# voutcn/megahit

Measured on NVIDIA H100. Metric: sorted (k+1)-mer edges/sec at k=27 on 150bp reads, higher is better.
Workload: dtype u32

## Files before the change

### megahit_b200/csrc/mhb_part.cuh

```cuda
#pragma once
#include "mhb_sort3.cuh"

namespace mhb {

__device__ __forceinline__ u32 atom_shared_inc_ret(u32 *p) {
  u32 old;
  asm volatile("atom.shared.add.u32 %0, [%1], 1;" : "=r"(old) : "r"(smem_u32(p)) : "memory");
  return old;
}

template <int WR>
struct PartCfg {
  static constexpr int THREADS = 384;
  static constexpr int IPT = SortGeom<WR>::IPT;
  static constexpr int TILE = THREADS * IPT;
  static constexpr size_t SMEM = 256 * 8  + 4 * 256 * 4  + 16 * 4 + (size_t)TILE * WR * 4;
  static constexpr size_t SMEM_OWNER_HIST = SMEM + 16 * 256 * 4;
};

template <int WR, bool OWNER_LUT, bool HAS_NEXT>
__global__ void __launch_bounds__(PartCfg<WR>::THREADS, 2)
    k_part_unstable(const u32 *__restrict__ in, u64 n, u32 num_tiles, int byte_idx,
                    const u64 *__restrict__ bin_addr ,
                    unsigned long long *gcursor , u32 *tile_counter,
                    u64 *next_hist, int next_byte, const uint8_t *__restrict__ digit_lut) {
  constexpr bool OWNER_HIST = OWNER_LUT && HAS_NEXT;
  using C = PartCfg<WR>;
  constexpr int THREADS = C::THREADS, IPT = C::IPT, TILE = C::TILE;
  extern __shared__ __align__(16) unsigned char smem_raw[];
  u64 *s_base = reinterpret_cast<u64 *>(smem_raw);
  u32 *s_cnt = reinterpret_cast<u32 *>(s_base + 256);
  u32 *s_off = s_cnt + 256;
  u32 *s_cur = s_off + 256;
  u32 *s_next = s_cur + 256;
  u32 *s_misc = s_next + 256;
  u32 *s_recs = s_misc + 16;
  u32 *s_onext = s_recs + (size_t)C::TILE * WR;
  __shared__ uint8_t s_lut[OWNER_LUT ? 256 : 1];
  const u32 tid = threadIdx.x, lane = tid & 31, warp = tid >> 5;
  const u32 widx = (u32)(WR - 1 - (byte_idx >> 2)), bsel = (u32)(byte_idx & 3);
  const u32 nwidx = (u32)(WR - 1 - (next_byte >> 2)), nbsel = (u32)(next_byte & 3);
  for (int i = tid; i < 256; i += THREADS) {
    s_cnt[i] = 0;
    s_next[i] = 0;
  }
  if constexpr (OWNER_HIST) {
    for (int i = tid; i < 16 * 256; i += THREADS) s_onext[i] = 0;
  }
  if constexpr (OWNER_LUT) {
    for (int i = tid; i < 256; i += THREADS) s_lut[i] = digit_lut[i];
  }
  if (tid == 0) s_misc[0] = atomicAdd(tile_counter, 1u);
  __syncthreads();
  u32 tile = s_misc[0];
  while (tile < num_tiles) {
    u32 next_ticket = 0;
    if (tid == 0) next_ticket = atomicAdd(tile_counter, 1u);
    const u64 tile_base = (u64)tile * TILE;
    const u32 valid = tile_base + TILE <= n ? (u32)TILE : (u32)(n - tile_base);
    u32 r[IPT][WR];
    u32 dg[IPT];
    const u32 wbase = warp * 32 * IPT + lane;
#pragma unroll
    for (int i = 0; i < IPT; ++i) {
      const u32 p = wbase + (u32)i * 32;
      if (p < valid) ld_rec_pinned<WR>(in, tile_base + p, r[i]);
    }
#pragma unroll
    for (int i = 0; i < IPT; ++i) {
      const u32 p = wbase + (u32)i * 32;
      u32 d = 0;
      if (p < valid) {
        d = rec_digit<WR>(r[i], widx, bsel);
        if constexpr (OWNER_LUT) d = s_lut[d];
        red_shared_inc(&s_cnt[d]);
      }
      dg[i] = d;
    }
    __syncthreads();
    if (tid < 256) {
      const u32 c = s_cnt[tid];
      const unsigned long long g = c ? atomicAdd(&gcursor[tid], (unsigned long long)c) : 0ull;
      u32 inc = c;
#pragma unroll
      for (int dd = 1; dd < 32; dd <<= 1) {
        const u32 t = __shfl_up_sync(0xffffffffu, inc, dd);
        if (lane >= (u32)dd) inc += t;
      }
      if (lane == 31) s_misc[4 + warp] = inc;
      s_off[tid] = inc - c;
      s_base[tid] = bin_addr[tid] + g * (u64)(WR * 4);
    }
    __syncthreads();
    if (tid < 256) {
      u32 add = 0;
#pragma unroll
      for (int w = 0; w < 7; ++w) add += (warp > (u32)w) ? s_misc[4 + w] : 0u;
      const u32 o = s_off[tid] + add;
      s_off[tid] = o;
      s_cur[tid] = o;
    }
    if (tid == 0) s_misc[0] = next_ticket;
    __syncthreads();
#pragma unroll
    for (int i = 0; i < IPT; ++i) {
      const u32 p = wbase + (u32)i * 32;
      if (p < valid) st_shared_rec<WR>(s_recs, atom_shared_inc_ret(&s_cur[dg[i]]), r[i]);
    }
    __syncthreads();
    const u32 next_tile = s_misc[0];
#pragma unroll
    for (int i = 0; i < IPT; ++i) {
      const u32 p = (u32)i * THREADS + tid;
      if (p < valid) {
        u32 q[WR];
        ld_rec<WR>(s_recs, p, q);
        u32 dd = rec_digit<WR>(q, widx, bsel);
        if constexpr (OWNER_LUT) dd = s_lut[dd];
        st_global_rec<WR>(s_base[dd] + (u64)(p - s_off[dd]) * (WR * 4), q);
        if constexpr (OWNER_HIST) red_shared_inc(&s_onext[(dd & 15u) * 256 + rec_digit<WR>(q, nwidx, nbsel)]);
        else if constexpr (HAS_NEXT) red_shared_inc(&s_next[rec_digit<WR>(q, nwidx, nbsel)]);
      }
    }
    for (int i = tid; i < 256; i += THREADS) s_cnt[i] = 0;
    __syncthreads();
    tile = next_tile;
  }
  if constexpr (OWNER_HIST) {
    for (int i = tid; i < 16 * 256; i += THREADS)
      if (s_onext[i]) atomicAdd((unsigned long long *)&next_hist[i], (unsigned long long)s_onext[i]);
  } else if constexpr (HAS_NEXT) {
    for (int i = tid; i < 256; i += THREADS)
      if (s_next[i]) atomicAdd((unsigned long long *)&next_hist[i], (unsigned long long)s_next[i]);
  }
}

}
```

### megahit_b200/csrc/mhb_sortdisp.cu

```cuda
#include <cuda_runtime.h>
#include <stdio.h>
#include <stdlib.h>
#include <string.h>

#include "mhb.h"
#include "mhb_common.cuh"
#include "mhb_kernels.cuh"
#include "mhb_sort3.cuh"
#include "mhb_part.cuh"

using namespace mhb;

template <int WR>
static u64 sort_tiles(u64 n) {
  return (n + SortGeom<WR>::TILE - 1) / SortGeom<WR>::TILE;
}
static u64 sort_num_tiles(u64 n, u32 words) {
#define M(WW) \
  if (words == WW) return sort_tiles<WW>(n);
  MHB_FOR_WR(M)
#undef M
  return 0;
}
static constexpr size_t kSortHeadBytes = (size_t)(72 + 1) * 256 * 8  + 256 * 8  + 128 * 4 + 256 * 8 ;

extern "C" size_t mhb_sort_workspace_bytes(uint64_t n, uint32_t words) {
  return kSortHeadBytes + (size_t)sort_num_tiles(n, words) * 256 * 8 + 256;
}

template <int WR>
static int launch_radix_pass(cudaStream_t st, const u32 *in, u64 n, int byte_idx, const u64 *bin_base,
                             u64 *lookback, u32 *tile_counter, u64 *next_hist, int next_byte, u32 epoch) {
  using G = SortGeom<WR>;
  static int blocks_per_sm = 0;
  if (!blocks_per_sm) {
    CK(cudaFuncSetAttribute(k_radix_pass3<WR, true>, cudaFuncAttributeMaxDynamicSharedMemorySize, (int)G::SMEM));
    CK(cudaFuncSetAttribute(k_radix_pass3<WR, false>, cudaFuncAttributeMaxDynamicSharedMemorySize, (int)G::SMEM));
    CK(cudaOccupancyMaxActiveBlocksPerMultiprocessor(&blocks_per_sm, k_radix_pass3<WR, true>, G::THREADS, G::SMEM));
    if (blocks_per_sm < 1) return mhb_set_error(MHB_ERR_CUDA, "radix pass kernel (WR=%d) does not fit an SM", WR);
    if (getenv("MHB_VERBOSE")) fprintf(stderr, "[mhb] radix pass WR=%d: %d threads x %d rec, %zu B smem, %d CTA/SM\n", WR, G::THREADS, G::IPT, G::SMEM, blocks_per_sm);
  }
  const u64 tiles = sort_tiles<WR>(n);
  u64 grid = (u64)blocks_per_sm * sm_count();
  if (grid > tiles) grid = tiles;
  if (next_hist)
    k_radix_pass3<WR, true><<<(int)grid, G::THREADS, G::SMEM, st>>>(in, n, (u32)tiles, byte_idx, bin_base, lookback,
                                                                     tile_counter, next_hist, next_byte, epoch);
  else
    k_radix_pass3<WR, false><<<(int)grid, G::THREADS, G::SMEM, st>>>(in, n, (u32)tiles, byte_idx, bin_base, lookback,
                                                                      tile_counter, nullptr, 0, epoch);
  CK_LAUNCH();
  return MHB_OK;
}

template <int WR, bool OWNER_LUT>
static int launch_part_unstable(cudaStream_t st, const u32 *in, u64 n, int byte_idx, const u64 *bin_base,
                                unsigned long long *gcursor, u32 *tile_counter, u64 *next_hist, int next_byte,
                                const uint8_t *lut) {
  using C = PartCfg<WR>;
  constexpr size_t SMEM_HIST = OWNER_LUT ? C::SMEM_OWNER_HIST : C::SMEM;
  static int bps = 0;
  if (!bps) {
    CK(cudaFuncSetAttribute(k_part_unstable<WR, OWNER_LUT, true>, cudaFuncAttributeMaxDynamicSharedMemorySize, (int)SMEM_HIST));
    CK(cudaFuncSetAttribute(k_part_unstable<WR, OWNER_LUT, false>, cudaFuncAttributeMaxDynamicSharedMemorySize, (int)C::SMEM));
    CK(cudaOccupancyMaxActiveBlocksPerMultiprocessor(&bps, k_part_unstable<WR, OWNER_LUT, true>, C::THREADS, SMEM_HIST));
    if (bps < 1) return mhb_set_error(MHB_ERR_CUDA, "partition pass (WR=%d) does not fit an SM", WR);
    if (getenv("MHB_VERBOSE")) fprintf(stderr, "[mhb] unstable partition pass WR=%d owner=%d: %d threads x %d rec, %zu B smem, %d CTA/SM\n", WR, (int)OWNER_LUT, C::THREADS, C::IPT, SMEM_HIST, bps);
  }
  const u64 tiles = (n + C::TILE - 1) / C::TILE;
  u64 grid = (u64)bps * sm_count();
  if (grid > tiles) grid = tiles;
  if (next_hist)
    k_part_unstable<WR, OWNER_LUT, true><<<(int)grid, C::THREADS, SMEM_HIST, st>>>(in, n, (u32)tiles, byte_idx, bin_base, gcursor,
                                                                                   tile_counter, next_hist, next_byte, lut);
  else
    k_part_unstable<WR, OWNER_LUT, false><<<(int)grid, C::THREADS, C::SMEM, st>>>(in, n, (u32)tiles, byte_idx, bin_base, gcursor,
                                                                                  tile_counter, nullptr, 0, lut);
  CK_LAUNCH();
  return MHB_OK;
}

#ifdef MHB_SORT_TIMELINE
extern "C" int mhb_debug_set_sort_timeline(unsigned long long *dev_buf, unsigned long long rows) {
  CK(cudaMemcpyToSymbol(g_sort_timeline, &dev_buf, sizeof(dev_buf)));
  CK(cudaMemcpyToSymbol(g_sort_timeline_rows, &rows, sizeof(rows)));
  return MHB_OK;
}
#endif

namespace {
struct SortTrace {
  cudaEvent_t ev[74];
  bool created = false;
  uint32_t n_passes = 0, words = 0;
  uint64_t n = 0;
};
SortTrace g_trace[4];
uint64_t g_trace_seq = 0;
}

static int sort_records_core(void *stream, uint32_t *a, uint32_t *b, uint64_t n, uint32_t words, const uint8_t *bytes,
                             uint32_t n_bytes, const uint64_t *first_hist, void *ws, size_t ws_bytes, int *result_in_b,
                             double *pass_ms_host, int relaxed, bool trace);
int mhb_sort_records_impl(void *stream, uint32_t *a, uint32_t *b, uint64_t n, uint32_t words, const uint8_t *bytes,
                          uint32_t n_bytes, const uint64_t *first_hist, void *ws, size_t ws_bytes, int *result_in_b,
                          double *pass_ms_host) {
  return sort_records_core(stream, a, b, n, words, bytes, n_bytes, first_hist, ws, ws_bytes, result_in_b, pass_ms_host, 1, true);
}
int mhb_sort_records_ex(void *stream, uint32_t *a, uint32_t *b, uint64_t n, uint32_t words, const uint8_t *bytes,
                        uint32_t n_bytes, const uint64_t *first_hist, void *ws, size_t ws_bytes, int *result_in_b,
                        double *pass_ms_host, int relaxed) {
  return sort_records_core(stream, a, b, n, words, bytes, n_bytes, first_hist, ws, ws_bytes, result_in_b, pass_ms_host, relaxed, true);
}
int mhb_sort_records_untraced(void *stream, uint32_t *a, uint32_t *b, uint64_t n, uint32_t words, const uint8_t *bytes,
                              uint32_t n_bytes, const uint64_t *first_hist, void *ws, size_t ws_bytes, int *result_in_b) {
  return sort_records_core(stream, a, b, n, words, bytes, n_bytes, first_hist, ws, ws_bytes, result_in_b, nullptr, 1, false);
}
static int sort_records_core(void *stream, uint32_t *a, uint32_t *b, uint64_t n, uint32_t words, const uint8_t *bytes,
                             uint32_t n_bytes, const uint64_t *first_hist, void *ws, size_t ws_bytes, int *result_in_b,
                             double *pass_ms_host, int relaxed, bool trace) {
  if (pass_ms_host && !trace) return mhb_set_error(MHB_ERR_ARG, "per-pass times need a traced sort");
  if (words < 1 || words > 17 || n_bytes > 72 || !result_in_b)
    return mhb_set_error(MHB_ERR_ARG, "bad sort geometry (words=%u n_bytes=%u)", words, n_bytes);
  *result_in_b = 0;
  if (n == 0 || n_bytes == 0) return MHB_OK;
  if (ws_bytes < mhb_sort_workspace_bytes(n, words)) return mhb_set_error(MHB_ERR_ARG, "sort workspace too small");
  if (n >= (1ull << 53)) return mhb_set_error(MHB_ERR_ARG, "too many records");
  cudaStream_t st = (cudaStream_t)stream;
  u64 *hist = (u64 *)ws;
  u64 *bin_base = hist + (72 + 1) * 256;
  u32 *tile_counter = (u32 *)(bin_base + 256);
  unsigned long long *gcursor = (unsigned long long *)(tile_counter + 128);
  u64 *lookback = (u64 *)((char *)ws + kSortHeadBytes);
  CK(cudaMemsetAsync(ws, 0, mhb_sort_workspace_bytes(n, words), st));
  if (first_hist) {
    CK(cudaMemcpyAsync(hist, first_hist, 256 * 8, cudaMemcpyDeviceToDevice, st));
  } else {
#define M(WW) \
  if (words == WW) k_hist_byte<WW><<<sm_count() * 4, 256, 0, st>>>(a, n, bytes[0], hist);
    MHB_FOR_WR(M)
#undef M
    CK_LAUNCH();
  }
  SortTrace *tr = nullptr;
  if (trace) {
    tr = &g_trace[g_trace_seq++ & 3];
    if (!tr->created) {
      for (int i = 0; i < 74; ++i) CK(cudaEventCreate(&tr->ev[i]));
      tr->created = true;
    }
    tr->n_passes = n_bytes;
    tr->words = words;
    tr->n = n;
    CK(cudaEventRecord(tr->ev[0], st));
  }
  u32 *in = a, *out = b;
  for (u32 p = 0; p < n_bytes; ++p) {
    k_hist_scan256<<<1, 256, 0, st>>>(hist + (u64)p * 256, bin_base, (u64)(uintptr_t)out, words * 4);
    CK_LAUNCH();
    u64 *next_hist = p + 1 < n_bytes ? hist + (u64)(p + 1) * 256 : nullptr;
    const int next_byte = p + 1 < n_bytes ? bytes[p + 1] : 0;
    int rc = MHB_ERR_ARG;
    if (p == 0 && relaxed && words == 2) rc = launch_part_unstable<2, false>(st, in, n, bytes[p], bin_base, gcursor, tile_counter + p, next_hist, next_byte, nullptr);
    else if (p == 0 && relaxed && words == 3) rc = launch_part_unstable<3, false>(st, in, n, bytes[p], bin_base, gcursor, tile_counter + p, next_hist, next_byte, nullptr);
    else {
#define M(WW) \
  if (words == WW) rc = launch_radix_pass<WW>(st, in, n, bytes[p], bin_base, lookback, tile_counter + p, next_hist, next_byte, p + 1);
      MHB_FOR_WR(M)
#undef M
    }
    if (rc) return rc;
    if (tr) CK(cudaEventRecord(tr->ev[p + 1], st));
    u32 *t = in;
    in = out;
    out = t;
  }
  *result_in_b = (in == b) ? 1 : 0;
  if (pass_ms_host) {
    CK(cudaEventSynchronize(tr->ev[n_bytes]));
    for (u32 p = 0; p < n_bytes; ++p) {
      float ms = 0;
      CK(cudaEventElapsedTime(&ms, tr->ev[p], tr->ev[p + 1]));
      pass_ms_host[p] = ms;
    }
  }
  return MHB_OK;
}

int hist_byte(void *stream, const uint32_t *recs, uint64_t n, uint32_t words, int byte, uint64_t *hist) {
  if (words < 1 || words > 17 || byte < 0 || byte >= (int)(4 * words)) return mhb_set_error(MHB_ERR_ARG, "bad geometry");
  if (n == 0) return MHB_OK;
  cudaStream_t st = (cudaStream_t)stream;
#define M(WW) \
  if (words == WW) k_hist_byte<WW><<<sm_count() * 4, 256, 0, st>>>(recs, n, byte, hist);
  MHB_FOR_WR(M)
#undef M
  CK_LAUNCH();
  return MHB_OK;
}

static int partition_scatter_impl(void *stream, const uint32_t *recs, uint64_t n, uint32_t words, int byte,
                                  const uint8_t *owner_of_byte_dev, const uint64_t *bin_addr_dev, void *ws, size_t ws_bytes,
                                  int next_byte, uint64_t *owner_next_hist) {
  if (words < 1 || words > 17 || byte < 0 || byte >= (int)(4 * words)) return mhb_set_error(MHB_ERR_ARG, "bad geometry");
  if (!owner_of_byte_dev) return mhb_set_error(MHB_ERR_ARG, "the partition pass needs an owner table");
  if (n == 0) return MHB_OK;
  if (ws_bytes < kSortHeadBytes) return mhb_set_error(MHB_ERR_ARG, "sort workspace too small");
  cudaStream_t st = (cudaStream_t)stream;
  u32 *tile_counter = (u32 *)((u64 *)ws + (72 + 1) * 256 + 256);
  unsigned long long *gcursor = (unsigned long long *)(tile_counter + 128);
  CK(cudaMemsetAsync(ws, 0, kSortHeadBytes, st));
  int rc = MHB_ERR_ARG;
#define M(WW)                                                                                                        \
  if (words == WW)                                                                                                   \
    rc = launch_part_unstable<WW, true>(st, recs, n, byte, bin_addr_dev, gcursor, tile_counter, owner_next_hist, next_byte, \
                                        owner_of_byte_dev);
  MHB_FOR_WR(M)
#undef M
  return rc;
}
extern "C" int mhb_partition_scatter(void *stream, const uint32_t *recs, uint64_t n, uint32_t words, int byte,
                                     const uint8_t *owner_of_byte_dev, const uint64_t *bin_addr_dev, void *ws,
                                     size_t ws_bytes) {
  return partition_scatter_impl(stream, recs, n, words, byte, owner_of_byte_dev, bin_addr_dev, ws, ws_bytes, 0, nullptr);
}
extern "C" int mhb_partition_scatter_hist(void *stream, const uint32_t *recs, uint64_t n, uint32_t words, int byte,
                                          const uint8_t *owner_of_byte_dev, const uint64_t *bin_addr_dev, void *ws,
                                          size_t ws_bytes, int next_byte, uint64_t *owner_next_hist) {
  if (!owner_next_hist || next_byte < 0 || next_byte >= (int)(4 * words))
    return mhb_set_error(MHB_ERR_ARG, "bad owner-histogram arguments");
  return partition_scatter_impl(stream, recs, n, words, byte, owner_of_byte_dev, bin_addr_dev, ws, ws_bytes, next_byte,
                                owner_next_hist);
}

extern "C" int mhb_dev_malloc(void **ptr, size_t bytes) {
  CK(cudaMalloc(ptr, bytes));
  return MHB_OK;
}
extern "C" int mhb_dev_free(void *ptr) {
  CK(cudaFree(ptr));
  return MHB_OK;
}
extern "C" int mhb_ipc_export(const void *dev_ptr, uint8_t *handle64) {
  static_assert(sizeof(cudaIpcMemHandle_t) == 64, "handle size");
  cudaIpcMemHandle_t h;
  CK(cudaIpcGetMemHandle(&h, const_cast<void *>(dev_ptr)));
  memcpy(handle64, &h, 64);
  return MHB_OK;
}
extern "C" int mhb_ipc_open(const uint8_t *handle64, void **peer_ptr) {
  cudaIpcMemHandle_t h;
  memcpy(&h, handle64, 64);
  CK(cudaIpcOpenMemHandle(peer_ptr, h, cudaIpcMemLazyEnablePeerAccess));
  return MHB_OK;
}
extern "C" int mhb_ipc_close(void *peer_ptr) {
  CK(cudaIpcCloseMemHandle(peer_ptr));
  return MHB_OK;
}

extern "C" int mhb_sort_pass_ms(int back, double *pass_ms, uint32_t max_passes, uint32_t *n_passes, uint64_t *n_records,
                                uint32_t *words) {
  if (back < 0 || back > 3 || (uint64_t)back >= g_trace_seq) return mhb_set_error(MHB_ERR_ARG, "no such sort in the trace ring");
  SortTrace &tr = g_trace[(g_trace_seq - 1 - back) & 3];
  CK(cudaEventSynchronize(tr.ev[tr.n_passes]));
  for (u32 p = 0; p < tr.n_passes && p < max_passes; ++p) {
    float ms = 0;
    CK(cudaEventElapsedTime(&ms, tr.ev[p], tr.ev[p + 1]));
    pass_ms[p] = ms;
  }
  if (n_passes) *n_passes = tr.n_passes;
  if (n_records) *n_records = tr.n;
  if (words) *words = tr.words;
  return MHB_OK;
}

extern "C" int mhb_sort_records(void *stream, uint32_t *a, uint32_t *b, uint64_t n, uint32_t words,
                                const uint8_t *bytes, uint32_t n_bytes, const uint64_t *first_hist, void *ws,
                                size_t ws_bytes, int *result_in_b) {
  return mhb_sort_records_ex(stream, a, b, n, words, bytes, n_bytes, first_hist, ws, ws_bytes, result_in_b, nullptr, 0);
}

extern "C" int mhb_sort_records_relaxed(void *stream, uint32_t *a, uint32_t *b, uint64_t n, uint32_t words,
                                        const uint8_t *bytes, uint32_t n_bytes, const uint64_t *first_hist, void *ws,
                                        size_t ws_bytes, int *result_in_b) {
  return mhb_sort_records_ex(stream, a, b, n, words, bytes, n_bytes, first_hist, ws, ws_bytes, result_in_b, nullptr, 1);
}
```

Baseline: 18.69 billion.

## Prefetch next partition tile into shared memory with bulk async copy

Adds a second shared-memory buffer and uses mbarrier-tracked bulk global-to-shared copies to prefetch the next tile while the current one is scattered, replacing per-thread global loads for full aligned tiles. Tile size per thread is enlarged and the launch bound drops to one block per SM. The aim is to hide global load latency behind the scatter phase. Doubled shared memory and the lower minimum-blocks hint may cut occupancy, and the single barrier relies on the staging buffer being consumed before the next issue.

```diff
diff --git a/megahit_b200/csrc/mhb_part.cuh b/megahit_b200/csrc/mhb_part.cuh
--- a/megahit_b200/csrc/mhb_part.cuh
+++ b/megahit_b200/csrc/mhb_part.cuh
@@ -12,18 +12,32 @@
 template <int WR>
 struct PartCfg {
   static constexpr int THREADS = 384;
-  static constexpr int IPT = SortGeom<WR>::IPT;
+  static constexpr int MIN_BLOCKS = 1;
+  static constexpr int IPT = WR == 1 ? 28 : 56 / WR;
   static constexpr int TILE = THREADS * IPT;
-  static constexpr size_t SMEM = 256 * 8  + 4 * 256 * 4  + 16 * 4 + (size_t)TILE * WR * 4;
+  static constexpr u32 TILE_BYTES = (u32)TILE * WR * 4;
+  static constexpr size_t SMEM = 256 * 8  + 4 * 256 * 4  + 16 * 4 + 16  +
+                                 2 * (size_t)TILE_BYTES ;
   static constexpr size_t SMEM_OWNER_HIST = SMEM + 16 * 256 * 4;
 };
 
+template <int WR>
+__device__ __forceinline__ bool part_tile_staged(int stage, u32 tile, u64 n) {
+  return stage && (u64)(tile + 1) * PartCfg<WR>::TILE <= n;
+}
+template <int WR>
+__device__ __forceinline__ void part_stage_tile(u32 *s_stage, u64 *bar, const u32 *in, u32 tile) {
+  constexpr u32 B = PartCfg<WR>::TILE_BYTES;
+  mbar_expect_tx(bar, B);
+  bulk_g2s(s_stage, in + (u64)tile * PartCfg<WR>::TILE * WR, B, bar);
+}
+
 template <int WR, bool OWNER_LUT, bool HAS_NEXT>
-__global__ void __launch_bounds__(PartCfg<WR>::THREADS, 2)
+__global__ void __launch_bounds__(PartCfg<WR>::THREADS, PartCfg<WR>::MIN_BLOCKS)
     k_part_unstable(const u32 *__restrict__ in, u64 n, u32 num_tiles, int byte_idx,
                     const u64 *__restrict__ bin_addr ,
                     unsigned long long *gcursor , u32 *tile_counter,
-                    u64 *next_hist, int next_byte, const uint8_t *__restrict__ digit_lut) {
+                    u64 *next_hist, int next_byte, const uint8_t *__restrict__ digit_lut, int stage) {
   constexpr bool OWNER_HIST = OWNER_LUT && HAS_NEXT;
   using C = PartCfg<WR>;
   constexpr int THREADS = C::THREADS, IPT = C::IPT, TILE = C::TILE;
@@ -34,8 +48,10 @@
   u32 *s_cur = s_off + 256;
   u32 *s_next = s_cur + 256;
   u32 *s_misc = s_next + 256;
-  u32 *s_recs = s_misc + 16;
-  u32 *s_onext = s_recs + (size_t)C::TILE * WR;
+  u64 *s_bar = reinterpret_cast<u64 *>(s_misc + 16);
+  u32 *s_recs = s_misc + 20;
+  u32 *s_stage = s_recs + (size_t)C::TILE * WR;
+  u32 *s_onext = s_stage + (size_t)C::TILE * WR;
   __shared__ uint8_t s_lut[OWNER_LUT ? 256 : 1];
   const u32 tid = threadIdx.x, lane = tid & 31, warp = tid >> 5;
   const u32 widx = (u32)(WR - 1 - (byte_idx >> 2)), bsel = (u32)(byte_idx & 3);
@@ -50,9 +66,16 @@
   if constexpr (OWNER_LUT) {
     for (int i = tid; i < 256; i += THREADS) s_lut[i] = digit_lut[i];
   }
-  if (tid == 0) s_misc[0] = atomicAdd(tile_counter, 1u);
+  if (tid == 0) {
+    mbar_init(s_bar, 1);
+    mbar_fence_init();
+    const u32 t0 = atomicAdd(tile_counter, 1u);
+    s_misc[0] = t0;
+    if (t0 < num_tiles && part_tile_staged<WR>(stage, t0, n)) part_stage_tile<WR>(s_stage, s_bar, in, t0);
+  }
   __syncthreads();
   u32 tile = s_misc[0];
+  u32 phase = 0;
   while (tile < num_tiles) {
     u32 next_ticket = 0;
     if (tid == 0) next_ticket = atomicAdd(tile_counter, 1u);
@@ -61,10 +84,17 @@
     u32 r[IPT][WR];
     u32 dg[IPT];
     const u32 wbase = warp * 32 * IPT + lane;
+    if (part_tile_staged<WR>(stage, tile, n)) {
+      mbar_wait(s_bar, phase);
+      phase ^= 1u;
 #pragma unroll
-    for (int i = 0; i < IPT; ++i) {
-      const u32 p = wbase + (u32)i * 32;
-      if (p < valid) ld_rec_pinned<WR>(in, tile_base + p, r[i]);
+      for (int i = 0; i < IPT; ++i) ld_rec<WR>(s_stage, wbase + (u32)i * 32, r[i]);
+    } else {
+#pragma unroll
+      for (int i = 0; i < IPT; ++i) {
+        const u32 p = wbase + (u32)i * 32;
+        if (p < valid) ld_rec_pinned<WR>(in, tile_base + p, r[i]);
+      }
     }
 #pragma unroll
     for (int i = 0; i < IPT; ++i) {
@@ -78,6 +108,8 @@
       dg[i] = d;
     }
     __syncthreads();
+    if (tid == 0 && next_ticket < num_tiles && part_tile_staged<WR>(stage, next_ticket, n))
+      part_stage_tile<WR>(s_stage, s_bar, in, next_ticket);
     if (tid < 256) {
       const u32 c = s_cnt[tid];
       const unsigned long long g = c ? atomicAdd(&gcursor[tid], (unsigned long long)c) : 0ull;
diff --git a/megahit_b200/csrc/mhb_sortdisp.cu b/megahit_b200/csrc/mhb_sortdisp.cu
--- a/megahit_b200/csrc/mhb_sortdisp.cu
+++ b/megahit_b200/csrc/mhb_sortdisp.cu
@@ -64,18 +64,19 @@
     CK(cudaFuncSetAttribute(k_part_unstable<WR, OWNER_LUT, true>, cudaFuncAttributeMaxDynamicSharedMemorySize, (int)SMEM_HIST));
     CK(cudaFuncSetAttribute(k_part_unstable<WR, OWNER_LUT, false>, cudaFuncAttributeMaxDynamicSharedMemorySize, (int)C::SMEM));
     CK(cudaOccupancyMaxActiveBlocksPerMultiprocessor(&bps, k_part_unstable<WR, OWNER_LUT, true>, C::THREADS, SMEM_HIST));
-    if (bps < 1) return mhb_set_error(MHB_ERR_CUDA, "partition pass (WR=%d) does not fit an SM", WR);
+    if (bps < C::MIN_BLOCKS) return mhb_set_error(MHB_ERR_CUDA, "partition pass (WR=%d) does not fit an SM", WR);
     if (getenv("MHB_VERBOSE")) fprintf(stderr, "[mhb] unstable partition pass WR=%d owner=%d: %d threads x %d rec, %zu B smem, %d CTA/SM\n", WR, (int)OWNER_LUT, C::THREADS, C::IPT, SMEM_HIST, bps);
   }
   const u64 tiles = (n + C::TILE - 1) / C::TILE;
   u64 grid = (u64)bps * sm_count();
   if (grid > tiles) grid = tiles;
+  const int stage = ((uintptr_t)in & 15u) == 0;
   if (next_hist)
     k_part_unstable<WR, OWNER_LUT, true><<<(int)grid, C::THREADS, SMEM_HIST, st>>>(in, n, (u32)tiles, byte_idx, bin_base, gcursor,
-                                                                                   tile_counter, next_hist, next_byte, lut);
+                                                                                   tile_counter, next_hist, next_byte, lut, stage);
   else
     k_part_unstable<WR, OWNER_LUT, false><<<(int)grid, C::THREADS, C::SMEM, st>>>(in, n, (u32)tiles, byte_idx, bin_base, gcursor,
-                                                                                  tile_counter, nullptr, 0, lut);
+                                                                                  tile_counter, nullptr, 0, lut, stage);
   CK_LAUNCH();
   return MHB_OK;
 }
```

After: 18.94 billion (median of 6 runs). +1.3%, better.
